# cvg/diffmvs

Measured on AMD Instinct MI355X. Metric: depth-maps/sec (640x512, 5 src views), higher is better.
Workload: dtype f32

## Files before the change

diffmvs_amd/_lib.py:

```python
from __future__ import annotations

import ctypes as C
import os

PKG = os.path.dirname(os.path.abspath(__file__))
HIP_LIB_PATH = os.environ.get("DMVS_LIB") or os.path.join(PKG, "libdmvs_hip.so")

ACT_NONE, ACT_RELU, ACT_SIGMOID, ACT_TANH, ACT_SILU = range(5)
IN_PLAIN, IN_UPSAMPLE2, IN_UNSHUFFLE2, IN_ZEROINSERT2 = range(4)
LAYOUT_NCHW, LAYOUT_NHWC, LAYOUT_NHWC_BF16, LAYOUT_NHWC_F16 = 0, 1, 2, 3
DTYPE_F32, DTYPE_BF16, DTYPE_F16, DTYPE_F32_PLAIN = 0, 1, 2, 3
ARITH_F32, ARITH_BF16, ARITH_SPLIT = 0, 1, 2
EW_DEPTH_TO_DISP, EW_DISP_TO_DEPTH = 0, 1

_P = C.c_void_p
_I = C.c_int32
_F = C.c_float


class Conv2dDesc(C.Structure):
    _fields_ = [
        ("in0", _P), ("in1", _P), ("mul0", _P), ("weight", _P), ("scale", _P), ("shift", _P),
        ("residual", _P), ("gru_z", _P), ("gru_h", _P), ("out", _P), ("gn_stats", _P), ("out_mul", _P),
        ("B", _I), ("c0", _I), ("c1", _I), ("Hin", _I), ("Win", _I), ("Hout", _I), ("Wout", _I),
        ("cout", _I), ("cout_pad", _I), ("kh", _I), ("kw", _I), ("stride", _I), ("pad_h", _I), ("pad_w", _I),
        ("in_mode", _I), ("act", _I), ("res_mode", _I), ("res_after_act", _I),
        ("out_layout", _I), ("out_cstride", _I), ("out_coffset", _I), ("gn_groups", _I), ("post_scale", _F),
        ("gate_cstride", _I), ("arith", _I), ("tune", _I), ("out_mul_c0", _I), ("in0_cstride", _I), ("weight_split", _P),
    ]


class Conv3dDesc(C.Structure):
    _fields_ = [
        ("in_", _P), ("weight", _P), ("scale", _P), ("shift", _P), ("residual", _P), ("out", _P),
        ("B", _I), ("cin", _I), ("cout", _I), ("cout_pad", _I),
        ("Din", _I), ("Hin", _I), ("Win", _I), ("Dout", _I), ("Hout", _I), ("Wout", _I),
        ("stride", _I), ("transposed", _I), ("act", _I), ("tune", _I),
    ]


class GetCostDesc(C.Structure):
    _fields_ = [
        ("ref", _P), ("src", _P), ("rt", _P), ("inv_depth", _P), ("confidence", _P), ("view_w", _P),
        ("disp_min", _P), ("disp_max", _P), ("out_cost", _P), ("out_samples", _P), ("worklist", _P),
        ("B", _I), ("S", _I), ("C", _I), ("G", _I), ("n", _I), ("H", _I), ("W", _I), ("vw_shift", _I),
        ("cost_cstride", _I), ("cost_coffset", _I), ("samp_cstride", _I), ("samp_coffset", _I),
        ("interval", _F), ("min_radius", _F), ("max_radius", _F), ("feat_dtype", _I), ("tune", _I),
    ]


SIGNATURES = {
    "dmvs_abi_version": [],
    "dmvs_conv2d_f32": [C.POINTER(Conv2dDesc), _P],
    "dmvs_featurenet_stem_f32": [_P, _P, _P, _P, _P, _P, _P, _P, _I, _I, _I, _I, _P],
    "dmvs_featurenet_stem3_f32": [_P, _P, _P, _P, _P, _P, _P, _P, _P, _P, _P, _I, _I, _I, _I, _P],
    "dmvs_featurenet_conv1_pair_f32": [_P, _P, _P, _P, _P, _P, _P, _P, _I, _I, _I, _I, _P],
    "dmvs_featurenet_fpn_tail_f32": [_P, _P, _P, _P, _P, _P, _I, _I, _I, _I, _P],
    "dmvs_conv2d_wgrad_workspace_f32": [C.POINTER(Conv2dDesc), C.POINTER(C.c_int64)],
    "dmvs_conv2d_wgrad_f32": [C.POINTER(Conv2dDesc), _P, _P, _P, _P, C.c_int64, _P],
    "dmvs_conv3d_f32": [C.POINTER(Conv3dDesc), _P],
    "dmvs_conv3d_wgrad_workspace_f32": [C.POINTER(Conv3dDesc), C.POINTER(C.c_int64)],
    "dmvs_conv3d_wgrad_f32": [C.POINTER(Conv3dDesc), _P, _P, _P, _P, C.c_int64, _P],
    "dmvs_compose_proj_f32": [_P, _P, _I, _I, _P],
    "dmvs_warp_volume_f32": [_P, _P, _P, _P, _I, _I, _I, _I, _I, _I, _I, _P],
    "dmvs_getcost_quad_f32": [C.POINTER(GetCostDesc), _P],
    "dmvs_warp_corr_init_quad_f32": [_P, _P, _P, _P, _P, _P, _I, _I, _I, _I, _I, _I, _I, _I, _I, _I, _I, _P],
    "dmvs_warp_corr_init_bwd_f32": [_P, _P, _P, _P, _P, _P, _P, _P, _I, _I, _I, _I, _I, _I, _I, _I, _I, _I, _P],
    "dmvs_getcost_bwd_f32": [C.POINTER(GetCostDesc), _P, _P, _P, _P],
    "dmvs_view_aggregate_bwd_f32": [_P, _P, _P, _P, _P, _P, _I, _I, _I, _I, _P],
    "dmvs_view_aggregate_f32": [_P, _P, _P, _I, _I, _I, _I, _P],
    "dmvs_sigmoid_max_d_f32": [_P, _P, _I, _I, _I, _P],
    "dmvs_depth_regress_f32": [_P, _P, _P, _P, _P, _P, _I, _I, _I, _P],
    "dmvs_convex_upsample_f32": [_P, _P, _P, _P, _P, _P, _I, _I, _I, _I, _P],
    "dmvs_mask_upsample4_f32": [_P, _P, _P, _F, _P, _P, _P, _P, _P, _I, _I, _I, _I, _I, _P],
    "dmvs_groupnorm_silu_f32": [_P, _P, _P, _P, _P, _P, _P, _I, _I, _I, _I, _F, _P],
    "dmvs_groupnorm_apply_f32": [_P, _P, _P, _P, _P, _P, _P, _I, _I, _I, _I, _F, _P],
    "dmvs_delta_update_f32": [_P, _P, _P, _F, _P, _P, _P, _I, _I, _I, _I, _P],
    "dmvs_depth_convert_f32": [_P, _P, _P, _P, _I, _I, _I, _P],
    "dmvs_act_slice_f32": [_P, _P, _I, _I, _I, _I, _I, _I, _I, _I, _P],
    "dmvs_upsample_nearest_f32": [_P, _P, _I, _I, _I, _I, _P],
    "dmvs_nchw_to_nhwc_f32": [_P, _P, _I, _I, _I, _P],
    "dmvs_groupnorm_silu_bwd_workspace_f32": [_I, _I, _I, C.POINTER(C.c_int64)],
    "dmvs_groupnorm_silu_bwd_f32": [_P, _P, _P, _P, _P, _P, _P, _P, _P, _P, _P, C.c_int64, _I, _I, _I, _I, _F, _P],
    "dmvs_batchnorm_workspace_f32": [_I, _I, _I, _I, C.POINTER(C.c_int64)],
    "dmvs_batchnorm_train_fwd_f32": [_P, _P, _P, _P, _P, _P, _P, _P, _P, C.c_int64, _I, _I, _I, _I, _I, _F, _F, _I, _P],
    "dmvs_batchnorm_train_bwd_f32": [_P, _P, _P, _P, _P, _P, _P, _P, _P, _P, C.c_int64, _I, _I, _I, _I, _I, _I, _P],
    "dmvs_geo_consistency_f32": [_P, _P, _P, _P, _P, _I, _I, _F, _F, _P, _P, _I, _I, _I, _I, _I, _P],
    "dmvs_sumsq_f32": [_P, C.c_int64, _P, _P],
    "dmvs_adamw_step_f32": [_P, _P, _P, _P, C.c_int64, _F, _F, _F, _F, _F, _I, _F, _P, _F, _P],
    "dmvs_view_select_scores_f64": [_P, _P, _P, _P, _P, C.c_int64, C.c_int64, _P, _I, C.c_double, C.c_double, C.c_double, _P, _P, _P],
    "dmvs_cloud_nn_dist_f32": [_P, C.c_int64, _P, C.c_int64, _P, _P, C.c_int64, _P, C.c_double, _P, _F, _P, _P, _P],
    "dmvs_cloud_stats_f32": [_P, _P, C.c_int64, _F, _P, _I, C.c_double, _I, _P, _P],
    "dmvs_cloud_nn_index_f32": [_P, C.c_int64, _P, C.c_int64, _P, _P, C.c_int64, _P, C.c_double, _P, _F, _P, _P, _P, _P, _P],
    "dmvs_cloud_pair_moments_f64": [_P, C.c_int64, _P, _P, C.c_int64, _P, _P, _F, _P, _P, C.c_double, C.c_double, C.c_double, _I, _P, _P],
    "dmvs_cloud_crop_prism_f32": [_P, C.c_int64, _P, _P, _I, _I, C.c_double, C.c_double, _P, _P],
    "dmvs_depth_stats_f32": [_P, _P, _P, C.c_int64, C.c_int64, _P, _I, C.c_double, C.c_double, C.c_double, C.c_double, _I, _P, _P],
    "dmvs_cloud_splat_zmin_f32": [_P, C.c_int64, _P, _P, C.c_int64, _I, _I, C.c_double, C.c_double, C.c_double, _I, _I, _P, _P, _P, _P],
    "dmvs_cloud_splat_sum_f32": [_P, C.c_int64, _P, _P, C.c_int64, _I, _I, C.c_double, C.c_double, C.c_double, C.c_double, C.c_double, _I, _P, _P, _P, _P],
    "dmvs_depth_normals_f32": [_P, _P, _P, C.c_int64, _I, _I, _I, C.c_double, _I, _P, _P, _P],
    "dmvs_tsdf_integrate_f32": [_P, _P, _P, _P, C.c_int64, _I, _I, _I, _I, _I, _P, C.c_double, C.c_double, _I, _P, _P, _P, _P],
    "dmvs_tsdf_flags_u8": [_P, _P, _I, _I, _I, _I, _P, _P, _P],
    "dmvs_tsdf_vertices_f32": [_P, _P, _P, _I, _I, _I, _P, C.c_double, _P, _P, C.c_int64, _P, _P, _P],
    "dmvs_tsdf_faces_i32": [_P, _I, _I, _I, _P, _P, _P, C.c_int64, _P, _P],
}
VIEW_SELECT_MAX_IMAGES, VIEW_SELECT_MAX_LIST = 16384, 1 << 23
CLOUD_MAX_RINGS, CLOUD_MAX_KEY_BITS, CLOUD_MAX_THRESHOLDS = 1024, 62, 16
CLOUD_MOMENTS, CLOUD_MAX_POLYGON = 20, 256
DEPTH_MAX_THRESHOLDS, DEPTH_SLOTS = 8, 7
SPLAT_VIEW_CHUNK, SPLAT_VIEW_DOUBLES, SPLAT_SLOTS, SPLAT_MAX_RADIUS, SPLAT_NO_PRETEST = 8, 15, 4, 16, 0x1
NORMAL_MAX_RADIUS, NORMAL_CAM_DOUBLES, NORMAL_VIEW_CHUNK, NORMAL_SLOTS = 4, 27, 8, 4
TSDF_VIEW_CHUNK, TSDF_VIEW_DOUBLES, TSDF_MAX_VIEWS, TSDF_MAX_QUADS, TSDF_NO_CULL = 8, 12, 65535, 357913941, 0x1
ABI_VERSION = 4
TUNE_NO_WALK, TUNE_PIECES4, TUNE_NO_LEAN, TUNE_1X1_TILED, TUNE_NO_TALL, TUNE_TALL = 0x4, 0x8, 0x100, 0x200, 0x400, 0x800
TUNE3D_PIECES4, TUNE3D_S2_DIRECT, TUNE3D_NO_PAIR = 0x1, 0x2, 0x4
TUNE_SWEEP_GLOBAL = 0x1
TUNE_WGRAD_ACCUMULATE = 0x1000
TUNE_SPLIT_ALL = 0x20000
TUNE_STEM_EXACT = 0x40000


def tune_xcd_group(n: int) -> int:
    return (int(n) & 7) << 14


def tune3d_xcd_group(n: int) -> int:
    return (int(n) & 7) << 4
TUNE_BWD_INTERLEAVED, BWD_GATHER_INTERLEAVED = 0x1, 2


def tune_tile_wx(n: int) -> int:
    return n & 3


def tune_tile_mt(n: int) -> int:
    return (n & 7) << 4


class DmvsError(RuntimeError):
    pass

# ... 32 lines not shown
```

diffmvs_amd/build.py:

```python
from __future__ import annotations

import os
import subprocess
import sys

PKG = os.path.dirname(os.path.abspath(__file__))
ROOT = os.path.dirname(PKG)
CSRC = os.path.join(PKG, "csrc")
LIB = os.path.join(PKG, "libdmvs_hip.so")
PROBE_LIB = os.path.join(PKG, "libdmvs_probe.so")
PROBE_SOURCES = ["probe/getcost_probe.hip", "probe/random_line_gather.hip"]
SOURCES = ["conv2d_k33.hip", "conv2d_k55.hip", "conv2d_k77.hip", "conv2d_k15.hip", "conv2d.hip", "stem.hip", "stem3.hip", "conv1_pair.hip", "fpn_tail.hip", "conv3d.hip", "warp_quad.hip", "warp_bwd.hip", "warp_bwd_win.hip", "warp_init_bwd_win.hip", "misc.hip", "mask_upsample.hip", "optim.hip", "norm.hip", "fusion.hip", "view_select.hip", "cloud_eval.hip", "cloud_register.hip", "depth_eval.hip", "cloud_render.hip", "depth_normals.hip", "tsdf.hip"]


def _deps():
    out = [os.path.join(ROOT, "include", "dmvs.h"), os.path.join(ROOT, "include", "dmvs_probe.h")]
    for base, _, files in os.walk(CSRC):
        out += [os.path.join(base, f) for f in files]
    return out


def _stale() -> bool:
    if not os.path.exists(LIB) or not os.path.exists(PROBE_LIB):
        return True
    t = min(os.path.getmtime(LIB), os.path.getmtime(PROBE_LIB))
    return any(os.path.getmtime(d) > t for d in _deps())


def build_hip(force: bool = False, save_temps: bool = False, verbose: bool = True) -> str:
    if not force and not _stale():
        return LIB
    import time
    t_start = time.time()
    hipcc = os.environ.get("HIPCC", "/opt/rocm/bin/hipcc")
    flags = ["--offload-arch=gfx950", "-O3", "-std=c++17", "-fPIC",
             "-I", os.path.join(ROOT, "include"), "-I", CSRC,
             "-munsafe-fp-atomics",
             "-Wall", "-Wno-unused-function"]
    objdir = os.path.join(ROOT, "build", "temps" if save_temps else "obj")
    os.makedirs(objdir, exist_ok=True)
    if save_temps:
        flags += ["-save-temps=obj", "-Rpass-analysis=kernel-resource-usage"]

    hdr_t = max(os.path.getmtime(d) for d in _deps() if d.endswith(".h"))

    def compile_one(src):
        obj = os.path.join(objdir, src.replace("/", "_") + ".o")
        if not force and not save_temps and os.path.exists(obj) and os.path.getmtime(obj) > max(hdr_t, os.path.getmtime(os.path.join(CSRC, src))):
            return obj
        cmd = [hipcc] + flags + ["-c", os.path.join(CSRC, src), "-o", obj]
        if verbose:
            print("[diffmvs_amd.build]", " ".join(cmd), flush=True)
        t0 = time.time()
        subprocess.run(cmd, check=True, cwd=objdir if save_temps else ROOT)
        os.utime(obj, (t0, t0))
        return obj

    from concurrent.futures import ThreadPoolExecutor
    with ThreadPoolExecutor(max_workers=min(len(SOURCES), os.cpu_count() or 4)) as pool:
        objs = list(pool.map(compile_one, SOURCES + PROBE_SOURCES))
    for lib, lobjs in ((LIB, objs[:len(SOURCES)]), (PROBE_LIB, objs[len(SOURCES):])):
        link = [hipcc, "--offload-arch=gfx950", "-shared", "-fPIC"] + lobjs + ["-o", lib]
        if verbose:
            print("[diffmvs_amd.build]", " ".join(link), flush=True)
        subprocess.run(link, check=True, cwd=ROOT)
        os.utime(lib, (t_start, t_start))
    return LIB


if __name__ == "__main__":
    build_hip(force="--force" in sys.argv, save_temps="--save-temps" in sys.argv)
    print(LIB)
```

diffmvs_amd/engine.py:

```python
from __future__ import annotations

import math
import os
from typing import Callable, Dict, List, Optional

import torch
import torch.nn.functional as F

from . import ops as K
from .ops import Ops, PackedConv, pack_conv2d, pack_conv3d

_RATIOS = [4, 2, 1]
_MULTS = [(1,), (1, 2), (1, 2, 4)]


def _bn(sd, p):
    return {k: sd[f"{p}.{k}"] for k in ("weight", "bias", "running_mean", "running_var")}


def _cw(sd, p, **kw):
    return pack_conv2d(sd[p + ".conv.weight"], sd.get(p + ".conv.bias"),
                       bn=_bn(sd, p + ".bn") if (p + ".bn.weight") in sd else None, **kw)


def pack_feature(sd, p="feature", g4=False, feat_dtype=torch.float32):
    order = (lambda w: w[K.g4_channels(w.shape[0], feat_dtype).to(w.device)].contiguous()) if g4 else (lambda w: w)
    f = {"conv0.0": _cw(sd, p + ".conv0.0", pad=1), "conv0.1": _cw(sd, p + ".conv0.1", pad=1)}
    for i in (1, 2, 3):
        f[f"conv{i}.0"] = _cw(sd, f"{p}.conv{i}.0", stride=2, pad=2)
        f[f"conv{i}.1"], f[f"conv{i}.2"] = _cw(sd, f"{p}.conv{i}.1", pad=1), _cw(sd, f"{p}.conv{i}.2", pad=1)
    f["out1"] = pack_conv2d(order(sd[p + ".out1.weight"]))
    f["inner1"] = pack_conv2d(sd[p + ".inner1.weight"], sd[p + ".inner1.bias"])
    f["out2"] = pack_conv2d(order(sd[p + ".out2.weight"]), pad=1)
    if (p + ".out3.weight") in sd:
        f["inner2"] = pack_conv2d(sd[p + ".inner2.weight"], sd[p + ".inner2.bias"])
        f["out3"] = pack_conv2d(order(sd[p + ".out3.weight"]), pad=1)
    return f


STEM_FUSE_DEFAULT = "1"


def stem3_applies(o: Ops, x):
    return (o.conv_arith == K.ARITH_SPLIT and os.environ.get("DMVS_STEM_FUSE", STEM_FUSE_DEFAULT) != "0" and
            o.featurenet_stem3_supported(x))


CONV1_PAIR_DEFAULT = "1"


def conv1_pair_applies(o: Ops, c1):
    return (o.conv_arith == K.ARITH_SPLIT and os.environ.get("DMVS_CONV1_PAIR", CONV1_PAIR_DEFAULT) != "0" and
            o.conv1_pair_supported(c1) and c1.shape[3] >= K.Ops.CONV1_PAIR_STRIP)


FPN_TAIL_DEFAULT = "1"


def fpn_tail_applies(o: Ops, f, c2, c3, layout, feat_dtype):
    return (o.conv_arith == K.ARITH_SPLIT and layout == K.LAYOUT_NHWC and feat_dtype == torch.float32 and "out3" not in f and
            os.environ.get("DMVS_FPN_TAIL", FPN_TAIL_DEFAULT) != "0" and o.fpn_tail_supported(c2, c3))


def run_feature(o: Ops, f, x, layout=K.LAYOUT_NHWC, feat_dtype=torch.float32):
    R = K.ACT_RELU
    if stem3_applies(o, x):
        c1 = o.featurenet_stem3(f["conv0.0"], f["conv0.1"], f["conv1.0"], x)
    else:
        c0 = o.featurenet_stem(f["conv0.0"], f["conv0.1"], x)
        c1 = o.conv2d(f["conv1.0"], c0, act=R)
    if conv1_pair_applies(o, c1):
        c1 = o.conv1_pair(f["conv1.1"], f["conv1.2"], c1)
    else:
        c1 = o.conv2d(f["conv1.2"], o.conv2d(f["conv1.1"], c1, act=R), act=R)
    c2 = o.conv2d(f["conv2.2"], o.conv2d(f["conv2.1"], o.conv2d(f["conv2.0"], c1, act=R), act=R), act=R)
    c3 = o.conv2d(f["conv3.2"], o.conv2d(f["conv3.1"], o.conv2d(f["conv3.0"], c2, act=R), act=R), act=R)
    out = {"stage1": o.conv2d(f["out1"], c3, out_layout=layout, out_dtype=feat_dtype)}
    if fpn_tail_applies(o, f, c2, c3, layout, feat_dtype):
        out["stage2"] = o.fpn_tail(f["inner1"], f["out2"], c2, c3)
        return out
    intra = o.conv2d(f["inner1"], c2, residual=c3, res_mode=K.IN_UPSAMPLE2)
    out["stage2"] = o.conv2d(f["out2"], intra, out_layout=layout, out_dtype=feat_dtype)
    if "out3" in f:
        intra = o.conv2d(f["inner2"], c1, residual=intra, res_mode=K.IN_UPSAMPLE2)
        out["stage3"] = o.conv2d(f["out3"], intra, out_layout=layout, out_dtype=feat_dtype)
    return out


def pack_context_trunk(sd, p="context"):
    c = {"conv1": _cw(sd, p + ".conv1", pad=1)}
    for li in (1, 2, 3):
        for bi in (0, 1):
            q = f"{p}.layer{li}.{bi}"
            c[f"{li}.{bi}.conv1"] = _cw(sd, q + ".conv1", stride=(2 if bi == 0 else 1), pad=1)
            c[f"{li}.{bi}.conv2"] = _cw(sd, q + ".conv2", pad=1)
            if bi == 0:
                c[f"{li}.{bi}.down"] = _cw(sd, q + ".downsample", stride=2, pad=1)
    return c


def run_context_trunk(o: Ops, c, x):
    R = K.ACT_RELU
    x = o.conv2d(c["conv1"], x, act=R)
    taps = {}
    for li in (1, 2, 3):
        y = o.conv2d(c[f"{li}.0.conv1"], x, act=R)
        xd = o.conv2d(c[f"{li}.0.down"], x)
        x = o.conv2d(c[f"{li}.0.conv2"], y, residual=xd, act=R)
        y = o.conv2d(c[f"{li}.1.conv1"], x, act=R)
        x = o.conv2d(c[f"{li}.1.conv2"], y, residual=x, act=R)
        taps[3 - li] = x
    return taps


def pack_pvw(sd, p):
    return (pack_conv3d(sd[p + ".conv.0.conv.weight"], bn=_bn(sd, p + ".conv.0.bn")),
            pack_conv3d(sd[p + ".conv.1.weight"], sd[p + ".conv.1.bias"]))


def run_pvw(o: Ops, pk, cor):
    N, _, D, H, W = cor.shape
    x = o.conv3d(pk[1], o.conv3d(pk[0], cor, act=K.ACT_RELU))
    return o.sigmoid_max_d(x.view(N, D, H, W))


def pack_costreg(sd, p):
    reg = {}
    for i, st in ((0, 1), (1, 1), (2, 2), (3, 1), (4, 2), (5, 1)):
        reg[i] = pack_conv3d(sd[f"{p}.conv{i}.conv.weight"], bn=_bn(sd, f"{p}.conv{i}.bn"), stride=st)
    for i in (6, 7):
        reg[i] = pack_conv3d(sd[f"{p}.conv{i}.conv.weight"], bn=_bn(sd, f"{p}.conv{i}.bn"), stride=2, transposed=True)
    reg["prob"] = pack_conv3d(sd[p + ".prob.weight"])
    return reg


def run_costreg(o: Ops, reg, x):
    R = K.ACT_RELU
    c1 = o.conv3d(reg[1], o.conv3d(reg[0], x, act=R), act=R)
    c3 = o.conv3d(reg[3], o.conv3d(reg[2], c1, act=R), act=R)
    x = o.conv3d(reg[5], o.conv3d(reg[4], c3, act=R), act=R)
    x = o.conv3d(reg[6], x, act=R, residual=c3)
    x = o.conv3d(reg[7], x, act=R, residual=c1)
    return o.conv3d(reg["prob"], x)


def pack_mask(sd, p):
    return (pack_conv2d(sd[p + ".0.weight"], sd[p + ".0.bias"], pad=1), pack_conv2d(sd[p + ".2.weight"], sd[p + ".2.bias"]))


def run_mask(o: Ops, pk, context, post_scale=0.25):
    return o.conv2d(pk[1], o.conv2d(pk[0], context, act=K.ACT_RELU), post_scale=post_scale)


def mask_head_fuses(pk, up_ratio) -> bool:
    return up_ratio == 4 and pk[1].cin == 64 and pk[1].cout == 144 and pk[1].scale is None and os.environ.get("DMVS_MASK_FUSE", "1") != "0"


def pack_gru(sd, p):
# ... 441 lines not shown
```

diffmvs_amd/ops.py:

```python
from __future__ import annotations

import ctypes as C
import os
from dataclasses import dataclass
from typing import Optional

import torch

from . import _lib
from ._lib import (ACT_NONE, ACT_RELU, ACT_SIGMOID, ACT_SILU, ACT_TANH, ARITH_BF16, ARITH_F32, ARITH_SPLIT, DTYPE_BF16, DTYPE_F16, DTYPE_F32, IN_PLAIN,
                   IN_UNSHUFFLE2, IN_UPSAMPLE2, IN_ZEROINSERT2, LAYOUT_NCHW, LAYOUT_NHWC, LAYOUT_NHWC_BF16, LAYOUT_NHWC_F16)

CONV_ARITH = {"fp32": ARITH_F32, "bf16": ARITH_BF16, "split": ARITH_SPLIT}
FEATURE_DTYPES = {"fp32": torch.float32, "bf16": torch.bfloat16, "fp16": torch.float16}
_DTYPE_CODE = {torch.float32: DTYPE_F32, torch.bfloat16: DTYPE_BF16, torch.float16: DTYPE_F16}
_NHWC_LAYOUT = {torch.float32: LAYOUT_NHWC, torch.bfloat16: LAYOUT_NHWC_BF16, torch.float16: LAYOUT_NHWC_F16}


def _round_up(x: int, m: int) -> int:
    return (x + m - 1) // m * m


@dataclass
class PackedConv:
# ... 291 lines not shown
        return y

    def _stem_launch(self, pc0: PackedConv, pc1: PackedConv, x, y, tune=None):
        N, cin, H, W = x.shape
        if not (cin == 3 and pc0.cin == 3 and pc0.cout == 8 and pc1.cin == 8 and pc1.cout == 8 and pc0.k == (3, 3) and
                pc1.k == (3, 3) and pc0.stride == 1 and pc1.stride == 1 and pc0.pad == (1, 1) and pc1.pad == (1, 1) and
                pc0.cout_pad == 8 and pc1.cout_pad == 8):
            raise _lib.DmvsError("featurenet_stem: expects the 3->8->8 3x3 stem of FeatureNet")
        tune = self.tune["stem"] if tune is None else tune
        if self.conv_arith != ARITH_SPLIT:
            tune |= _lib.TUNE_STEM_EXACT
        self._call("dmvs_featurenet_stem_f32", _ptr(x), _ptr(pc0.weight), _ptr(pc0.scale), _ptr(pc0.shift), _ptr(pc1.weight),
                   _ptr(pc1.scale), _ptr(pc1.shift), _ptr(y), N, H, W, tune, self.stream())

    @staticmethod
    def featurenet_stem3_supported(x):
        xs = x if isinstance(x, (list, tuple)) else [x]
        H, W = xs[0].shape[2], xs[0].shape[3]
        return H % 2 == 0 and W % 4 == 0 and 3 * H * W < 2 ** 31 and all(t.data_ptr() % 16 == 0 for t in xs)

    def featurenet_stem3(self, pc0: PackedConv, pc1: PackedConv, pc2: PackedConv, x, tune=None):
        xs = x if isinstance(x, (list, tuple)) else [x]
        self._chk(*xs)
        Bv, cin, H, W = xs[0].shape
        if not (cin == 3 and pc0.cin == 3 and pc0.cout == 8 and pc1.cin == 8 and pc1.cout == 8 and pc0.k == (3, 3) and
                pc1.k == (3, 3) and pc0.stride == 1 and pc1.stride == 1 and pc0.pad == (1, 1) and pc1.pad == (1, 1) and
                pc0.cout_pad == 8 and pc1.cout_pad == 8 and pc2.cin == 8 and pc2.cout == 16 and pc2.cout_pad == 16 and pc2.k == (5, 5) and
                pc2.stride == 2 and pc2.pad == (2, 2)):
            raise _lib.DmvsError("featurenet_stem3: expects the 3->8->8 3x3 stem of FeatureNet and its 8->16 5x5 stride-2 conv1.0")
        if not self.featurenet_stem3_supported(xs) or any(t.shape != xs[0].shape for t in xs):
            raise _lib.DmvsError(f"featurenet_stem3: needs even H, W % 4 == 0 and 16-byte aligned views of one shape, got {tuple(xs[0].shape)}")
        y = self.empty(len(xs) * Bv, 16, H // 2, W // 2)
        for v, xv in enumerate(xs):
            self._call("dmvs_featurenet_stem3_f32", _ptr(xv), _ptr(pc0.weight), _ptr(pc0.scale), _ptr(pc0.shift), _ptr(pc1.weight),
                       _ptr(pc1.scale), _ptr(pc1.shift), _ptr(pc2.weight), _ptr(pc2.scale), _ptr(pc2.shift), _ptr(y[v * Bv:(v + 1) * Bv]),
                       Bv, H, W, 0 if tune is None else tune, self.stream())
        return y

    CONV1_PAIR_STRIP, CONV1_PAIR_SEGMENT = 80, 64

    @staticmethod
    def conv1_pair_supported(x):
        return (x.dim() == 4 and x.shape[1] == 16 and x.shape[3] % 4 == 0 and 16 * x.shape[2] * x.shape[3] < 2 ** 31 and
                x.data_ptr() % 16 == 0)

    def conv1_pair(self, pc1: PackedConv, pc2: PackedConv, x, tune=0):
        self._chk(x)
        for pc in (pc1, pc2):
            if not (pc.cin == 16 and pc.cout == 16 and pc.cout_pad == 16 and pc.k == (3, 3) and pc.stride == 1 and pc.pad == (1, 1)):
                raise _lib.DmvsError("conv1_pair: expects the two 16->16 3x3 stride-1 layers of FeatureNet's conv1")
        if not self.conv1_pair_supported(x):
            raise _lib.DmvsError(f"conv1_pair: needs 16 channels, W % 4 == 0 and a 16-byte aligned tensor, got {tuple(x.shape)}")
        N, _, H, W = x.shape
        y = self.empty(N, 16, H, W)
        self._call("dmvs_featurenet_conv1_pair_f32", _ptr(x), _ptr(split_weights(pc1)), _ptr(pc1.scale), _ptr(pc1.shift),
                   _ptr(split_weights(pc2)), _ptr(pc2.scale), _ptr(pc2.shift), _ptr(y), N, H, W, tune, self.stream())
        return y

    FPN_TAIL_STRIP, FPN_TAIL_SEGMENT = 32, 64

    @staticmethod
    def fpn_tail_supported(c2, c3):
        if not (c2.dim() == 4 and c3.dim() == 4 and c2.dtype == torch.float32 and c3.dtype == torch.float32):
            return False
        N, C, H, W = c2.shape
        return (C == 32 and H % 2 == 0 and W % 8 == 0 and H > 0 and W > 0 and tuple(c3.shape) == (N, 64, H // 2, W // 2) and
                64 * H * W < 2 ** 31 and c2.is_contiguous() and c3.is_contiguous() and c2.data_ptr() % 16 == 0 and c3.data_ptr() % 16 == 0)

    def fpn_tail(self, pc_inner: PackedConv, pc_out: PackedConv, c2, c3, tune=0):
        self._chk(c2, c3)
        if not (pc_inner.cin == 32 and pc_inner.cout == 64 and pc_inner.cout_pad == 64 and pc_inner.k == (1, 1) and pc_inner.stride == 1 and
                pc_inner.pad == (0, 0) and pc_inner.scale is None and pc_out.cin == 64 and pc_out.cout == 32 and pc_out.cout_pad == 32 and
                pc_out.k == (3, 3) and pc_out.stride == 1 and pc_out.pad == (1, 1) and pc_out.scale is None and pc_out.shift is None):
            raise _lib.DmvsError("fpn_tail: expects FeatureNet's inner1 (32->64 1x1, bias) and out2 (64->32 3x3, no bias)")
        if not self.fpn_tail_supported(c2, c3):
            raise _lib.DmvsError(f"fpn_tail: needs c2 [N,32,H,W] and c3 [N,64,H/2,W/2] with even H, W % 8 == 0, contiguous and 16-byte aligned, "
                                 f"got {tuple(c2.shape)} and {tuple(c3.shape)}")
        N, _, H, W = c2.shape
        y = self.empty(N, H, W, 32)
        self._call("dmvs_featurenet_fpn_tail_f32", _ptr(c2), _ptr(c3), _ptr(pc_inner.weight), _ptr(pc_inner.shift), _ptr(split_weights(pc_out)),
                   _ptr(y), N, H, W, tune, self.stream())
        return y

    def conv2d_wgrad(self, pc: PackedConv, x0, grad_out, x1=None, *, mul0=None, in_mode=IN_PLAIN, want_bias=False, tune=None,
                     into_gw=None, into_gb=None):
        self._chk(x0, x1, mul0, grad_out, into_gw, into_gb)
        B = x0.shape[0]
        if in_mode == IN_PLAIN:
            c0, Hin, Win = x0.shape[1], x0.shape[2], x0.shape[3]
        elif in_mode in (IN_UPSAMPLE2, IN_ZEROINSERT2):
            c0, Hin, Win = x0.shape[1], x0.shape[2] * 2, x0.shape[3] * 2
        else:
            c0, Hin, Win = x0.shape[1] * 4, x0.shape[2] // 2, x0.shape[3] // 2
        c1 = 0 if x1 is None else x1.shape[1]
        kh, kw = pc.k
        Hout, Wout = grad_out.shape[2], grad_out.shape[3]
        acc = into_gw is not None
        if acc and (tuple(into_gw.shape) != (pc.cout, pc.cin, kh, kw) or (want_bias and (into_gb is None or tuple(into_gb.shape) != (pc.cout,)))):
            raise _lib.DmvsError("conv2d_wgrad: into_gw / into_gb do not have the gradient's shape")
        gw = into_gw if acc else self.empty(pc.cout, pc.cin, kh, kw)
        gb = (into_gb if acc else self.empty(pc.cout)) if want_bias else None
        d = _lib.Conv2dDesc(
            in0=_ptr(x0), in1=_ptr(x1), mul0=_ptr(mul0), weight=None, scale=None, shift=None, residual=None, gru_z=None,
            gru_h=None, out=None, gn_stats=None, gn_groups=0, B=B, c0=c0, c1=c1, Hin=Hin, Win=Win, Hout=Hout, Wout=Wout,
            cout=pc.cout, cout_pad=pc.cout_pad, kh=kh, kw=kw, stride=pc.stride, pad_h=pc.pad[0], pad_w=pc.pad[1],
            in_mode=in_mode, act=ACT_NONE, res_mode=IN_PLAIN, res_after_act=0, out_layout=LAYOUT_NCHW,
            out_cstride=pc.cout, out_coffset=0, post_scale=1.0, gate_cstride=0, arith=ARITH_F32,
            tune=((self.tune["conv2d"] & _lib.TUNE_PIECES4) if tune is None else tune) | (_lib.TUNE_WGRAD_ACCUMULATE if acc else 0))
        nbytes = C.c_int64(0)
        self._call("dmvs_conv2d_wgrad_workspace_f32", C.byref(d), C.byref(nbytes))
        ws = self.empty(nbytes.value // 4)
        self._call("dmvs_conv2d_wgrad_f32", C.byref(d), _ptr(grad_out), _ptr(gw), _ptr(gb), _ptr(ws), nbytes.value, self.stream())
        if self.timers is not None and "dmvs_conv2d_wgrad_f32" in self.timers:
            self.timers.setdefault("_wgrad_flops", []).append(2.0 * B * Hout * Wout * pc.cout * pc.cin * kh * kw)
        return (gw, gb) if want_bias else gw

    def conv3d(self, pc: PackedConv, x, *, act=ACT_NONE, residual=None, out=None, tune=None):
        self._chk(x, residual, out)
        B, cin, Din, Hin, Win = x.shape
        assert cin == pc.cin
        if pc.transposed:
            Dout, Hout, Wout = 2 * Din, 2 * Hin, 2 * Win
        else:
            s = pc.stride
            Dout, Hout, Wout = (Din - 1) // s + 1, (Hin - 1) // s + 1, (Win - 1) // s + 1
        if out is None:
            out = self.empty(B, pc.cout, Dout, Hout, Wout)
        d = _lib.Conv3dDesc(in_=_ptr(x), weight=_ptr(pc.weight), scale=_ptr(pc.scale), shift=_ptr(pc.shift),
                            residual=_ptr(residual), out=_ptr(out), B=B, cin=cin, cout=pc.cout, cout_pad=pc.cout_pad,
                            Din=Din, Hin=Hin, Win=Win, Dout=Dout, Hout=Hout, Wout=Wout, stride=pc.stride,
                            transposed=int(pc.transposed), act=act, tune=(self.tune["conv3d"] if tune is None else tune))
        self._call("dmvs_conv3d_f32", C.byref(d), self.stream())
        return out

    def conv3d_wgrad(self, x, grad_out, cout, stride, want_bias=False):
        self._chk(x, grad_out)
        B, cin, Din, Hin, Win = x.shape
        Dout, Hout, Wout = grad_out.shape[2:]
        gw = self.empty(cout, cin, 3, 3, 3)
        gb = self.empty(cout) if want_bias else None
        d = _lib.Conv3dDesc(in_=_ptr(x), weight=None, scale=None, shift=None, residual=None, out=None, B=B, cin=cin,
                            cout=cout, cout_pad=_pad_cout(cout), Din=Din, Hin=Hin, Win=Win, Dout=Dout, Hout=Hout, Wout=Wout,
                            stride=stride, transposed=0, act=ACT_NONE)
        nbytes = C.c_int64(0)
        self._call("dmvs_conv3d_wgrad_workspace_f32", C.byref(d), C.byref(nbytes))
        ws = self.empty(nbytes.value // 4)
        self._call("dmvs_conv3d_wgrad_f32", C.byref(d), _ptr(grad_out), _ptr(gw), _ptr(gb), _ptr(ws), nbytes.value, self.stream())
        return (gw, gb) if want_bias else gw

    def compose_proj(self, proj):
        self._chk(proj)
        B, V = proj.shape[0], proj.shape[1]
        out = self.empty(B, V - 1, 12)
        self._call("dmvs_compose_proj_f32", _ptr(proj), _ptr(out), B, V, self.stream())
        return out

    def warp_corr_init_quad(self, ref, src, rt, disp_min, disp_max, D, G=4, tune=None, plain=False):
        self._chk(rt, disp_min, disp_max)
        fdt = self._chk_feat(ref, src)
        if plain and fdt == DTYPE_F32:
            fdt = _lib.DTYPE_F32_PLAIN
        B, H, W, Cc = ref.shape
        S, _, Hs, Ws, _ = src.shape
        out = self.empty(B, S, G, D, H, W)
        self._call("dmvs_warp_corr_init_quad_f32", _ptr(ref), _ptr(src), _ptr(rt), _ptr(disp_min), _ptr(disp_max), _ptr(out),
                   B, S, Cc, G, D, H, W, Hs, Ws, fdt, self.tune["sweep"] if tune is None else tune, self.stream())
# ... 521 lines not shown
```

include/dmvs.h:

```cpp
#ifndef DMVS_H
#define DMVS_H

#include <stdint.h>

#ifdef __cplusplus
extern "C" {
#endif

#define DMVS_ABI_VERSION 4
#define DMVS_EINVAL (-22)

enum { DMVS_ACT_NONE = 0, DMVS_ACT_RELU = 1, DMVS_ACT_SIGMOID = 2, DMVS_ACT_TANH = 3, DMVS_ACT_SILU = 4 };
enum { DMVS_IN_PLAIN = 0, DMVS_IN_UPSAMPLE2 = 1 , DMVS_IN_UNSHUFFLE2 = 2 ,
       DMVS_IN_ZEROINSERT2 = 3  };
enum { DMVS_LAYOUT_NCHW = 0, DMVS_LAYOUT_NHWC = 1,
       DMVS_LAYOUT_NHWC_BF16 = 2, DMVS_LAYOUT_NHWC_F16 = 3 };
enum { DMVS_DTYPE_F32 = 0 , DMVS_DTYPE_BF16 = 1, DMVS_DTYPE_F16 = 2 ,
       DMVS_DTYPE_F32_PLAIN = 3  };

int dmvs_abi_version(void);

#define DMVS_ARITH_F32 0
#define DMVS_ARITH_BF16 1
#define DMVS_ARITH_SPLIT 2

#define DMVS_TUNE_TILE_WX(n) ((n) & 3)
#define DMVS_TUNE_NO_WALK 0x4
#define DMVS_TUNE_PIECES4 0x8
#define DMVS_TUNE_TILE_MT(n) (((n) & 7) << 4)
#define DMVS_TUNE_1X1_TILED 0x200
#define DMVS_TUNE_NO_LEAN 0x100
#define DMVS_TUNE_TALL(n) (((n) & 3) << 10)
#define DMVS_TUNE_STEM_EXACT 0x40000
#define DMVS_TUNE_SPLIT_ALL 0x20000
#define DMVS_TUNE_XCD_GROUP(n) (((n) & 7) << 14)

typedef struct dmvs_conv2d_desc {
    const float* in0;
    const float* in1;
    const float* mul0;
    const float* weight;
    const float* scale;
    const float* shift;
    const float* residual;
    const float* gru_z;
    const float* gru_h;
    float* out;
    double* gn_stats;
    const float* out_mul;
    int32_t B, c0, c1;
    int32_t Hin, Win;
    int32_t Hout, Wout;
    int32_t cout, cout_pad;
    int32_t kh, kw, stride, pad_h, pad_w;
    int32_t in_mode, act;
    int32_t res_mode;
    int32_t res_after_act;
    int32_t out_layout, out_cstride, out_coffset;
    int32_t gn_groups;
    float post_scale;
    int32_t gate_cstride;
    int32_t arith;
    int32_t tune;
    int32_t out_mul_c0;
    int32_t in0_cstride;
    const void* weight_split;
} dmvs_conv2d_desc;

int dmvs_conv2d_f32(const dmvs_conv2d_desc* d, void* stream);

int dmvs_featurenet_stem_f32(const float* x, const float* w0, const float* scale0, const float* shift0, const float* w1,
                             const float* scale1, const float* shift1, float* y, int32_t N, int32_t H, int32_t W, int32_t tune,
                             void* stream);

int dmvs_featurenet_stem3_f32(const float* x, const float* w0, const float* scale0, const float* shift0, const float* w1,
                              const float* scale1, const float* shift1, const float* w2, const float* scale2, const float* shift2,
                              float* y, int32_t N, int32_t H, int32_t W, int32_t tune, void* stream);

int dmvs_featurenet_conv1_pair_f32(const float* x, const void* wsplit1, const float* scale1, const float* shift1, const void* wsplit2,
                                   const float* scale2, const float* shift2, float* y, int32_t N, int32_t H, int32_t W, int32_t tune,
                                   void* stream);

int dmvs_featurenet_fpn_tail_f32(const float* c2, const float* c3, const float* w_inner, const float* b_inner, const void* wsplit_out,
                                 float* y, int32_t N, int32_t H, int32_t W, int32_t tune, void* stream);

#define DMVS_TUNE_WGRAD_ACCUMULATE 0x1000
int dmvs_conv2d_wgrad_workspace_f32(const dmvs_conv2d_desc* d, int64_t* bytes);
int dmvs_conv2d_wgrad_f32(const dmvs_conv2d_desc* d, const float* grad_out, float* gw, float* gb, float* workspace,
                          int64_t workspace_bytes, void* stream);

typedef struct dmvs_conv3d_desc {
    const float* in;
    const float* weight;
    const float* scale;
    const float* shift;
    const float* residual;
    float* out;
    int32_t B, cin, cout, cout_pad;
    int32_t Din, Hin, Win;
    int32_t Dout, Hout, Wout;
    int32_t stride;
    int32_t transposed;
    int32_t act;
    int32_t tune;
} dmvs_conv3d_desc;
#define DMVS_TUNE3D_PIECES4 0x1
#define DMVS_TUNE3D_S2_DIRECT 0x2
#define DMVS_TUNE3D_NO_PAIR 0x4
#define DMVS_TUNE3D_XCD_GROUP(n) (((n) & 7) << 4)

int dmvs_conv3d_f32(const dmvs_conv3d_desc* d, void* stream);

int dmvs_conv3d_wgrad_workspace_f32(const dmvs_conv3d_desc* d, int64_t* bytes);
int dmvs_conv3d_wgrad_f32(const dmvs_conv3d_desc* d, const float* grad_out, float* gw, float* gb, float* workspace,
                          int64_t workspace_bytes, void* stream);

int dmvs_compose_proj_f32(const float* proj, float* out, int32_t B, int32_t V, void* stream);

#define DMVS_GETCOST_TILE 16
#define DMVS_GETCOST_MAX_WINDOW_VIEWS 16
#define DMVS_GETCOST_WORKLIST_INTS(B, H, W) \
    (4 + 66 * (B) * (((H) + DMVS_GETCOST_TILE - 1) / DMVS_GETCOST_TILE) * (((W) + DMVS_GETCOST_TILE - 1) / DMVS_GETCOST_TILE))
typedef struct dmvs_getcost_desc {
    const float* ref;
    const float* src;
    const float* rt;
    const float* inv_depth;
    const float* confidence;
    const float* view_w;
    const float* disp_min;
    const float* disp_max;
    float* out_cost;
    float* out_samples;
    int32_t* worklist;
    int32_t B, S, C, G, n, H, W;
    int32_t vw_shift;
    int32_t cost_cstride, cost_coffset, samp_cstride, samp_coffset;
    float interval, min_radius, max_radius;
    int32_t feat_dtype;
    int32_t tune;
} dmvs_getcost_desc;

#define DMVS_TUNE_SWEEP_GLOBAL 0x1
int dmvs_getcost_quad_f32(const dmvs_getcost_desc* d, void* stream);
int dmvs_warp_corr_init_quad_f32(const void* ref, const void* src, const float* rt,
                                 const float* disp_min, const float* disp_max, float* out,
                                 int32_t B, int32_t S, int32_t C, int32_t G, int32_t D,
                                 int32_t H, int32_t W, int32_t Hs, int32_t Ws, int32_t feat_dtype, int32_t tune, void* stream);

int dmvs_warp_volume_f32(const float* src, const float* rt, const float* depth, float* out,
                         int32_t B, int32_t C, int32_t D, int32_t H, int32_t W, int32_t Hs, int32_t Ws,
                         void* stream);

#define DMVS_TUNE_BWD_INTERLEAVED 0x1
#define DMVS_BWD_GATHER_INTERLEAVED 2
int dmvs_warp_corr_init_bwd_f32(const float* ref, const float* src, const float* rt,
                                const float* disp_min, const float* disp_max, const float* gcor,
                                float* gref, float* gsrc, int32_t B, int32_t S, int32_t C, int32_t G,
                                int32_t D, int32_t H, int32_t W, int32_t Hs, int32_t Ws, int32_t gather, void* stream);
int dmvs_getcost_bwd_f32(const dmvs_getcost_desc* d, const float* gcost, float* gref, float* gsrc, void* stream);
int dmvs_view_aggregate_bwd_f32(const float* cor, const float* w, const float* out, const float* gout,
                                float* gcor, float* gw, int32_t B, int32_t S, int32_t GD, int32_t HW,
                                void* stream);

int dmvs_view_aggregate_f32(const float* cor, const float* w, float* out,
                            int32_t B, int32_t S, int32_t GD, int32_t HW, void* stream);

int dmvs_sigmoid_max_d_f32(const float* x, float* out, int32_t N, int32_t D, int32_t HW, void* stream);
// ... 136 lines not shown
```

Baseline: 1551.

## Add dedicated MFMA kernel for FeatureNet 5x5 stride-2 downsampling conv

Adds a specialized persistent kernel for the 16->32 5x5 stride-2 conv2.0 layer and routes to it by default when split-bf16 arithmetic is on. Input rows are streamed into LDS with async global-to-LDS loads and split into three bf16 parts held in a ring buffer. Output rows are computed with bf16 MFMA over a split-precision product, with part of the weights kept resident in registers, and the fused BN+ReLU applied on store. It replaces a generic conv2d launch for one layer of the feature network, which is only a small slice of the full depth pipeline, at the cost of a large amount of layer-specific code.

Result: faster. 1569, median of 6 (+1.2%).

```diff
diff --git a/diffmvs_amd/_lib.py b/diffmvs_amd/_lib.py
--- a/diffmvs_amd/_lib.py
+++ b/diffmvs_amd/_lib.py
@@ -56,6 +56,7 @@
     "dmvs_featurenet_stem3_f32": [_P, _P, _P, _P, _P, _P, _P, _P, _P, _P, _P, _I, _I, _I, _I, _P],
     "dmvs_featurenet_conv1_pair_f32": [_P, _P, _P, _P, _P, _P, _P, _P, _I, _I, _I, _I, _P],
     "dmvs_featurenet_fpn_tail_f32": [_P, _P, _P, _P, _P, _P, _I, _I, _I, _I, _P],
+    "dmvs_featurenet_down5_f32": [_P, _P, _P, _P, _P, _I, _I, _I, _I, _P],
     "dmvs_conv2d_wgrad_workspace_f32": [C.POINTER(Conv2dDesc), C.POINTER(C.c_int64)],
     "dmvs_conv2d_wgrad_f32": [C.POINTER(Conv2dDesc), _P, _P, _P, _P, C.c_int64, _P],
     "dmvs_conv3d_f32": [C.POINTER(Conv3dDesc), _P],
diff --git a/diffmvs_amd/build.py b/diffmvs_amd/build.py
--- a/diffmvs_amd/build.py
+++ b/diffmvs_amd/build.py
@@ -10,7 +10,7 @@
 LIB = os.path.join(PKG, "libdmvs_hip.so")
 PROBE_LIB = os.path.join(PKG, "libdmvs_probe.so")
 PROBE_SOURCES = ["probe/getcost_probe.hip", "probe/random_line_gather.hip"]
-SOURCES = ["conv2d_k33.hip", "conv2d_k55.hip", "conv2d_k77.hip", "conv2d_k15.hip", "conv2d.hip", "stem.hip", "stem3.hip", "conv1_pair.hip", "fpn_tail.hip", "conv3d.hip", "warp_quad.hip", "warp_bwd.hip", "warp_bwd_win.hip", "warp_init_bwd_win.hip", "misc.hip", "mask_upsample.hip", "optim.hip", "norm.hip", "fusion.hip", "view_select.hip", "cloud_eval.hip", "cloud_register.hip", "depth_eval.hip", "cloud_render.hip", "depth_normals.hip", "tsdf.hip"]
+SOURCES = ["conv2d_k33.hip", "conv2d_k55.hip", "conv2d_k77.hip", "conv2d_k15.hip", "conv2d.hip", "stem.hip", "stem3.hip", "conv1_pair.hip", "fpn_tail.hip", "down5.hip", "conv3d.hip", "warp_quad.hip", "warp_bwd.hip", "warp_bwd_win.hip", "warp_init_bwd_win.hip", "misc.hip", "mask_upsample.hip", "optim.hip", "norm.hip", "fusion.hip", "view_select.hip", "cloud_eval.hip", "cloud_register.hip", "depth_eval.hip", "cloud_render.hip", "depth_normals.hip", "tsdf.hip"]
 
 
 def _deps():
diff --git a/diffmvs_amd/csrc/down5.hip b/diffmvs_amd/csrc/down5.hip
--- /dev/null
+++ b/diffmvs_amd/csrc/down5.hip
@@ -0,0 +1,237 @@
+
+#include "dmvs_common.h"
+#include "dmvs_bf16.h"
+#include "dmvs_lds_poison.h"
+
+namespace {
+
+typedef float f32x4 __attribute__((ext_vector_type(4)));
+typedef uint32_t u32x4s __attribute__((ext_vector_type(4)));
+
+constexpr int PB = DMVS_BLOCK;
+constexpr int US = 32, UR = 64;
+constexpr int NPU = 2 * US + 3;
+constexpr int NP = NPU + 1;
+constexpr int SLOTS = 8, NCH = 2;
+constexpr int PLQ = SLOTS * NCH * NP;
+constexpr int RINGQ = 3 * PLQ;
+constexpr int SW = 2 * US + 8;
+constexpr int NPIECE = 4 * 16 * SW / 4;
+constexpr int NITEM = 4 * NCH * NPU;
+constexpr int NIT = (NITEM + PB - 1) / PB;
+constexpr int LDSF = RINGQ * 4 + NPIECE * 4;
+constexpr int NG = 7;
+constexpr int NSTEP = NCH * NG;
+constexpr int WR = 6;
+constexpr int WD = 2;
+
+__device__ __attribute__((aligned(16))) const float down5_zero16[4] = {0.0f, 0.0f, 0.0f, 0.0f};
+#define DMVS_LDS_P(p) ((__attribute__((address_space(3))) void*)(p))
+#ifdef DMVS_HOST_EMULATION
+#define DMVS_OPAQUE(v) ((void)0)
+#else
+#define DMVS_OPAQUE(v) asm volatile("" : "+v"(v))
+#endif
+
+__global__ void __launch_bounds__(PB) __attribute__((amdgpu_waves_per_eu(2, 2)))
+featurenet_down5_kernel(const float* __restrict__ x, const u32x4s* __restrict__ ws, const float* __restrict__ scale,
+                        const float* __restrict__ shift, float* __restrict__ y, int N, int H, int W, int nsx, int nsy) {
+    __shared__ __attribute__((aligned(16))) float lds[LDSF];
+    DMVS_LDS_POISON(lds);
+
+    const int tid = threadIdx.x, lane = tid & 63, wave = __builtin_amdgcn_readfirstlane(tid >> 6);
+    const int m = lane & 15, kq = lane >> 4;
+    const int Ho = H >> 1, Wo = W >> 1;
+    const int iplane = H * W, oplane = Ho * Wo;
+    const int nunits = nsx * nsy * N;
+
+    const int nt = wave & 1, rr = wave >> 1;
+    unsigned lwb = (unsigned)(kq * 32 + nt * 16 + m) * 16u;
+    auto wload = [&](int sp) -> u32x4s {
+        return *reinterpret_cast<const u32x4s*>(reinterpret_cast<const char*>(ws + sp * 128) + lwb);
+    };
+    const float sc = scale ? scale[16 * nt + m] : 1.0f, sh = shift ? shift[16 * nt + m] : 0.0f;
+    unsigned tapy = 0, tapx = 0;
+#pragma unroll
+    for (int g = 0; g < NG; ++g) {
+        const int t = min(4 * g + kq, 24);
+        tapy |= (unsigned)(t / 5) << (4 * g);
+        tapx |= (unsigned)(t % 5) << (4 * g);
+    }
+    const bool vec = (Wo & 3) == 0 && ((uintptr_t)y & 15) == 0;
+    u32x4s* const ring = reinterpret_cast<u32x4s*>(lds);
+    float* const st = lds + RINGQ * 4;
+
+    u32x4s wres[WR > 0 ? WR : 1][3];
+#pragma unroll
+    for (int s0 = 0; s0 < WR; ++s0)
+#pragma unroll
+        for (int pl = 0; pl < 3; ++pl) wres[s0][pl] = wload(s0 * 3 + pl);
+
+    int lm = m, ltid = tid;
+
+    for (int unit = blockIdx.x; unit < nunits; unit += gridDim.x) {
+        const int sx = unit % nsx;
+        const int uq = unit / nsx;
+        const int sy = uq % nsy, n = uq / nsy;
+        const int X0 = US * sx, Y0 = UR * sy;
+        const int Q = (min(UR, Ho - Y0) + 1) >> 1;
+        const float* const xb = x + (long)n * 16 * iplane;
+        float* const yb = y + (long)n * 32 * oplane;
+
+        auto stage = [&](int k, int lt) {
+#pragma unroll
+            for (int i = 0; i < (NPIECE + PB - 1) / PB; ++i) {
+                if (i * PB + wave * 64 < NPIECE) {
+                    const int e = i * PB + lt;
+                    const int li = e / (NPIECE / 4), rem = e - li * (NPIECE / 4);
+                    const int ch = rem / (SW / 4), pc = rem - ch * (SW / 4);
+                    const int row = 2 * Y0 - 3 + 4 * k + li, col = 2 * X0 - 4 + 4 * pc;
+                    const bool ok = row >= 0 && row < H && col >= 0 && col < W;
+                    const float* srcp = ok ? xb + (ch * iplane + row * W + col) : down5_zero16;
+                    float* dstp = st + (i * PB + wave * 64) * 4;
+                    __builtin_amdgcn_global_load_lds(srcp, DMVS_LDS_P(dstp), 16, 0, 0);
+                }
+            }
+        };
+        stage(0, ltid);
+        DMVS_DMA_BARRIER();
+
+        for (int j = 0; j < Q + 2; ++j) {
+            DMVS_OPAQUE(lm);
+            DMVS_OPAQUE(ltid);
+            DMVS_OPAQUE(lwb);
+            const bool do_out = j >= 2, do_in = j <= Q;
+            const int orow = Y0 + 2 * (j - 2) + rr;
+            f32x4 oacc[2] = {{0.0f, 0.0f, 0.0f, 0.0f}, {0.0f, 0.0f, 0.0f, 0.0f}};
+            if (do_out) {
+                auto qp_of = [&](int s) {
+                    const int c = s / NG, g = s - c * NG;
+                    const int slot = (2 * orow + 6 + (int)((tapy >> (4 * g)) & 7u)) & 7;
+                    return (slot * NCH + c) * NP + 2 * lm + (int)((tapx >> (4 * g)) & 7u);
+                };
+                u32x4s wq[WD + 1][3];
+                bf16x8 pq[2][2][3];
+#pragma unroll
+                for (int s0 = WR; s0 < WR + WD; ++s0)
+#pragma unroll
+                    for (int pl = 0; pl < 3; ++pl) wq[(s0 - WR) % (WD + 1)][pl] = wload(s0 * 3 + pl);
+                {
+                    const int qp = qp_of(0);
+#pragma unroll
+                    for (int grp = 0; grp < 2; ++grp)
+#pragma unroll
+                        for (int pl = 0; pl < 3; ++pl) pq[0][grp][pl] = __builtin_bit_cast(bf16x8, ring[pl * PLQ + qp + 32 * grp]);
+                }
+#pragma unroll
+                for (int s = 0; s < NSTEP; ++s) {
+                    const int pb = s & 1;
+                    __builtin_amdgcn_sched_barrier(0);
+                    if (s + WD >= WR + WD && s + WD < NSTEP) {
+#pragma unroll
+                        for (int pl = 0; pl < 3; ++pl) wq[(s + WD - WR) % (WD + 1)][pl] = wload((s + WD) * 3 + pl);
+                    }
+                    if (s + 1 < NSTEP) {
+                        const int qn = qp_of(s + 1);
+#pragma unroll
+                        for (int grp = 0; grp < 2; ++grp)
+#pragma unroll
+                            for (int pl = 0; pl < 3; ++pl) pq[pb ^ 1][grp][pl] = __builtin_bit_cast(bf16x8, ring[pl * PLQ + qn + 32 * grp]);
+                    }
+                    __builtin_amdgcn_sched_barrier(0);
+                    const u32x4s* const wcur = s < WR ? wres[s] : wq[(s - WR) % (WD + 1)];
+                    const bf16x8 wh = __builtin_bit_cast(bf16x8, wcur[0]), wm = __builtin_bit_cast(bf16x8, wcur[1]),
+                                 wlo = __builtin_bit_cast(bf16x8, wcur[2]);
+#pragma unroll
+                    for (int grp = 0; grp < 2; ++grp) oacc[grp] = dmvs_mfma_bf16(pq[pb][grp][2], wh, oacc[grp]);
+#pragma unroll
+                    for (int grp = 0; grp < 2; ++grp) oacc[grp] = dmvs_mfma_bf16(pq[pb][grp][0], wlo, oacc[grp]);
+#pragma unroll
+                    for (int grp = 0; grp < 2; ++grp) oacc[grp] = dmvs_mfma_bf16(pq[pb][grp][1], wm, oacc[grp]);
+#pragma unroll
+                    for (int grp = 0; grp < 2; ++grp) oacc[grp] = dmvs_mfma_bf16(pq[pb][grp][1], wh, oacc[grp]);
+#pragma unroll
+                    for (int grp = 0; grp < 2; ++grp) oacc[grp] = dmvs_mfma_bf16(pq[pb][grp][0], wm, oacc[grp]);
+#pragma unroll
+                    for (int grp = 0; grp < 2; ++grp) oacc[grp] = dmvs_mfma_bf16(pq[pb][grp][0], wh, oacc[grp]);
+                }
+                __builtin_amdgcn_sched_barrier(0);
+            }
+            u32x4s cv[NIT][3];
+            if (do_in) {
+#pragma unroll
+                for (int i = 0; i < NIT; ++i) {
+                    if (i * PB + wave * 64 < NITEM) {
+                        const int e = min(i * PB + ltid, NITEM - 1);
+                        const int li = e / (NCH * NPU), rem = e - li * (NCH * NPU);
+                        const int c = rem / NPU, p = rem - c * NPU;
+                        const float* sp = st + (li * 16 + c * 8) * SW + p + 2;
+                        float v[8];
+#pragma unroll
+                        for (int c8 = 0; c8 < 8; ++c8) v[c8] = sp[c8 * SW];
+                        bf16x8 h8, m8, l8;
+                        dmvs_split3_bf16x8(v, h8, m8, l8);
+                        cv[i][0] = __builtin_bit_cast(u32x4s, h8);
+                        cv[i][1] = __builtin_bit_cast(u32x4s, m8);
+                        cv[i][2] = __builtin_bit_cast(u32x4s, l8);
+                    }
+                }
+            }
+            DMVS_LDS_BARRIER();
+            if (j + 1 <= Q) stage(j + 1, ltid);
+            if (do_out && orow < Ho) {
+#pragma unroll
+                for (int grp = 0; grp < 2; ++grp) {
+                    const int ox = X0 + grp * 16 + 4 * kq;
+                    if (ox < Wo) {
+                        f32x4 v;
+#pragma unroll
+                        for (int r = 0; r < 4; ++r) v[r] = fmaxf(oacc[grp][r] * sc + sh, 0.0f);
+                        float* dst = yb + ((16 * nt + m) * oplane + orow * Wo + ox);
+                        if (vec) {
+                            *reinterpret_cast<f32x4*>(dst) = v;
+                        } else {
+#pragma unroll
+                            for (int r = 0; r < 4; ++r)
+                                if (ox + r < Wo) dst[r] = v[r];
+                        }
+                    }
+                }
+            }
+            if (do_in) {
+#pragma unroll
+                for (int i = 0; i < NIT; ++i) {
+                    const int e = i * PB + ltid;
+                    if (i * PB + wave * 64 < NITEM && e < NITEM) {
+                        const int li = e / (NCH * NPU), rem = e - li * (NCH * NPU);
+                        const int c = rem / NPU, p = rem - c * NPU;
+                        const int slot = (2 * Y0 - 3 + 4 * j + li + 8) & 7;
+                        u32x4s* const d = ring + (slot * NCH + c) * NP + p;
+                        d[0] = cv[i][0];
+                        d[PLQ] = cv[i][1];
+                        d[2 * PLQ] = cv[i][2];
+                    }
+                }
+            }
+            DMVS_DMA_BARRIER();
+        }
+    }
+}
+
+}
+
+extern "C" int dmvs_featurenet_down5_f32(const float* x, const void* wsplit, const float* scale, const float* shift, float* y, int32_t N,
+                                         int32_t H, int32_t W, int32_t tune, void* stream) {
+    if (!x || !wsplit || !y || N <= 0 || H <= 0 || W <= 0) return DMVS_EINVAL;
+    if ((H & 1) || (W & 3) || (long)16 * H * W >= (1L << 31)) return DMVS_EINVAL;
+    if ((((uintptr_t)x | (uintptr_t)wsplit) & 15) || ((uintptr_t)y & 3) || ((uintptr_t)scale & 3) || ((uintptr_t)shift & 3)) return DMVS_EINVAL;
+    const int nsx = (W / 2 + US - 1) / US, nsy = (H / 2 + UR - 1) / UR;
+    const long nunits = (long)nsx * nsy * N;
+    if (nunits >= (1L << 31)) return DMVS_EINVAL;
+    static const int resident = dmvs_resident_workgroups(reinterpret_cast<const void*>(featurenet_down5_kernel));
+    long grid = (tune & 0xffff) ? (tune & 0xffff) : resident;
+    if (grid > nunits) grid = nunits;
+    hipLaunchKernelGGL(featurenet_down5_kernel, dim3((unsigned)grid), dim3(PB), 0, (hipStream_t)stream, x,
+                       reinterpret_cast<const u32x4s*>(wsplit), scale, shift, y, N, H, W, nsx, nsy);
+    return dmvs_launch_status();
+}
diff --git a/diffmvs_amd/engine.py b/diffmvs_amd/engine.py
--- a/diffmvs_amd/engine.py
+++ b/diffmvs_amd/engine.py
@@ -62,6 +62,13 @@
             os.environ.get("DMVS_FPN_TAIL", FPN_TAIL_DEFAULT) != "0" and o.fpn_tail_supported(c2, c3))
 
 
+DOWN5_DEFAULT = "1"
+
+
+def down5_applies(o: Ops, c1):
+    return (o.conv_arith == K.ARITH_SPLIT and os.environ.get("DMVS_DOWN5", DOWN5_DEFAULT) != "0" and o.down5_supported(c1))
+
+
 def run_feature(o: Ops, f, x, layout=K.LAYOUT_NHWC, feat_dtype=torch.float32):
     R = K.ACT_RELU
     if stem3_applies(o, x):
@@ -73,7 +80,8 @@
         c1 = o.conv1_pair(f["conv1.1"], f["conv1.2"], c1)
     else:
         c1 = o.conv2d(f["conv1.2"], o.conv2d(f["conv1.1"], c1, act=R), act=R)
-    c2 = o.conv2d(f["conv2.2"], o.conv2d(f["conv2.1"], o.conv2d(f["conv2.0"], c1, act=R), act=R), act=R)
+    c2 = o.down5(f["conv2.0"], c1) if down5_applies(o, c1) else o.conv2d(f["conv2.0"], c1, act=R)
+    c2 = o.conv2d(f["conv2.2"], o.conv2d(f["conv2.1"], c2, act=R), act=R)
     c3 = o.conv2d(f["conv3.2"], o.conv2d(f["conv3.1"], o.conv2d(f["conv3.0"], c2, act=R), act=R), act=R)
     out = {"stage1": o.conv2d(f["out1"], c3, out_layout=layout, out_dtype=feat_dtype)}
     if fpn_tail_applies(o, f, c2, c3, layout, feat_dtype):
diff --git a/diffmvs_amd/ops.py b/diffmvs_amd/ops.py
--- a/diffmvs_amd/ops.py
+++ b/diffmvs_amd/ops.py
@@ -397,6 +397,28 @@
                    _ptr(y), N, H, W, tune, self.stream())
         return y
 
+    DOWN5_STRIP, DOWN5_SEGMENT = 32, 64
+
+    @staticmethod
+    def down5_supported(x):
+        if not (x.dim() == 4 and x.dtype == torch.float32):
+            return False
+        _, C_, H, W = x.shape
+        return (C_ == 16 and H > 0 and W > 0 and H % 2 == 0 and W % 4 == 0 and 16 * H * W < 2 ** 31 and x.is_contiguous() and
+                x.data_ptr() % 16 == 0)
+
+    def down5(self, pc: PackedConv, x, tune=0):
+        if not (pc.cin == 16 and pc.cout == 32 and pc.cout_pad == 32 and pc.k == (5, 5) and pc.stride == 2 and pc.pad == (2, 2)):
+            raise _lib.DmvsError("down5: expects a 16->32 5x5 stride-2 pad-2 layer (FeatureNet's conv2.0)")
+        if not self.down5_supported(x):
+            raise _lib.DmvsError(f"down5: needs [N,16,H,W] fp32 with even H, W % 4 == 0, contiguous and 16-byte aligned, got {tuple(x.shape)}")
+        self._chk(x)
+        N, _, H, W = x.shape
+        y = self.empty(N, 32, H // 2, W // 2)
+        self._call("dmvs_featurenet_down5_f32", _ptr(x), _ptr(split_weights(pc)), _ptr(pc.scale), _ptr(pc.shift), _ptr(y), N, H, W, tune,
+                   self.stream())
+        return y
+
     def conv2d_wgrad(self, pc: PackedConv, x0, grad_out, x1=None, *, mul0=None, in_mode=IN_PLAIN, want_bias=False, tune=None,
                      into_gw=None, into_gb=None):
         self._chk(x0, x1, mul0, grad_out, into_gw, into_gb)
diff --git a/include/dmvs.h b/include/dmvs.h
--- a/include/dmvs.h
+++ b/include/dmvs.h
@@ -84,6 +84,9 @@
 int dmvs_featurenet_fpn_tail_f32(const float* c2, const float* c3, const float* w_inner, const float* b_inner, const void* wsplit_out,
                                  float* y, int32_t N, int32_t H, int32_t W, int32_t tune, void* stream);
 
+int dmvs_featurenet_down5_f32(const float* x, const void* wsplit, const float* scale, const float* shift, float* y, int32_t N, int32_t H,
+                              int32_t W, int32_t tune, void* stream);
+
 #define DMVS_TUNE_WGRAD_ACCUMULATE 0x1000
 int dmvs_conv2d_wgrad_workspace_f32(const dmvs_conv2d_desc* d, int64_t* bytes);
 int dmvs_conv2d_wgrad_f32(const dmvs_conv2d_desc* d, const float* grad_out, float* gw, float* gb, float* workspace,
```
